# MP-Gadget/shenqi

Hardware: AMD Instinct MI355X
Metric: particle-steps/sec (grav+PM+SPH) at 256^3; rms force error vs ref (higher is better)
Workload: dtype f64

## Files before the change

include/shenqi_hip.h:

```cpp
#ifndef SHENQI_HIP_H
#define SHENQI_HIP_H

#include <stddef.h>
#include <stdint.h>

#ifdef __cplusplus
extern "C" {
#endif

#define SHQ_OK 0
#define SHQ_ERR_INVALID 1
#define SHQ_ERR_DEVICE 2
#define SHQ_ERR_NOMEM 3
#define SHQ_ERR_STATE 4
#define SHQ_ERR_NOCONV 5

#define SHQ_NGRAVTAB 512
#define SHQ_NMAXCHILD 8
#define SHQ_NODELISTLENGTH 4
#define SHQ_TIMEBINS 46

typedef struct shq_context shq_context;


// ... 371 lines not shown
int shq_bh_dynamics_download(shq_context *ctx, const shq_part_view *parts, const shq_bh_dyn_view *bh);
int shq_set_bh_reposition(shq_context *ctx, int enabled);
int shq_kick_bh(shq_context *ctx, const double gravkick[SHQ_TIMEBINS + 1], const int32_t *active, int64_t nactive);
int shq_grav_short_run(shq_context *ctx, const shq_grav_params *params, const int32_t *active,
                       int64_t nactive, int update_potential, int walk_mode);
int shq_grav_short_run_range(shq_context *ctx, const shq_grav_params *params, int64_t first, int64_t count,
                             int update_potential, int walk_mode);
int shq_set_walk_stats(shq_context *ctx, int level);
int shq_set_walk_launch(shq_context *ctx, int persist, int leaf_ring);
int shq_set_walk_sparse(shq_context *ctx, int enable);
int shq_walk_pair_lean(shq_context *ctx);
int shq_set_walk_overlap(shq_context *ctx, int mode);
int shq_set_walk_addr(shq_context *ctx, int mode);
int shq_walk_last_addr(shq_context *ctx, int *mode);
int shq_walk_addr32_fits(int64_t numnodes);
int shq_walk_pair_status(shq_context *ctx, int64_t *recovered_launches, int64_t *stack_high_water, int64_t *last_mopped_tasks);
int shq_set_walk_debug(shq_context *ctx, int pair_spin_max, int pair_stack_cap);
int shq_set_tree_debug(shq_context *ctx, int64_t initial_node_cap);
int shq_tree_build_attempts(shq_context *ctx, int *attempts);
int shq_direct_force_sample(shq_context *ctx, const double *sample_pos, int64_t ns, int64_t nsrc, double BoxSize, double G, double h,
                            int repeat, double *accel);
int shq_grav_short_download(shq_context *ctx, double (*accel)[3], double *potential,
                            int64_t *ninteractions, shq_walk_stats *stats);
typedef struct shq_grav_query {
    double Pos[3];
    int32_t NodeList[4];
    double OldAcc;
} shq_grav_query;
typedef struct shq_grav_result {
    double Acc[3];
    double Potential;
} shq_grav_result;
int shq_grav_short_secondary(shq_context *ctx, const shq_grav_params *params, const shq_grav_query *queries, int64_t nq,
                             shq_grav_result *results, int64_t *ninteractions, int update_potential);
typedef struct shq_data_index {
    int32_t Task;
    int32_t Index;
    int32_t NodeList[4];
// ... 980 lines not shown
```

shenqi_amd/capi.py:

```python
import ctypes as C
import os

import numpy as np

_HERE = os.path.dirname(os.path.abspath(__file__))
LIBDIR = os.environ.get("SHQ_LIBDIR") or os.path.join(_HERE, "lib")
DATADIR = os.path.join(_HERE, "data")

NGRAVTAB = 512
NMAXCHILD = 8
NOFIELD = C.c_size_t(-1).value

WALK_EXACT = 0
WALK_GROUP = 1
WALK_AUTO = 2
WALK_TREE_ORDER = 0x100
WALK_DEFER_POSTPROCESS = 0x200


class ShqError(RuntimeError):
    """Non-zero status from the library (the shim's endrun() equivalent)."""


def _load(name):
# ... 400 lines not shown
    getattr(hip, _f).restype = C.c_int
hip.shq_set_walk_stats.argtypes = [_vp, C.c_int]
hip.shq_set_walk_stats.restype = C.c_int
hip.shq_set_walk_launch.argtypes = [_vp, C.c_int, C.c_int]
hip.shq_set_walk_launch.restype = C.c_int
hip.shq_set_walk_sparse.argtypes = [_vp, C.c_int]
hip.shq_set_walk_sparse.restype = C.c_int
hip.shq_walk_pair_lean.argtypes = [_vp]
hip.shq_walk_pair_lean.restype = C.c_int
hip.shq_set_walk_overlap.argtypes = [_vp, C.c_int]
hip.shq_set_walk_overlap.restype = C.c_int
hip.shq_set_walk_addr.argtypes = [_vp, C.c_int]
hip.shq_set_walk_addr.restype = C.c_int
hip.shq_walk_last_addr.argtypes = [_vp, C.POINTER(C.c_int)]
hip.shq_walk_last_addr.restype = C.c_int
hip.shq_walk_addr32_fits.argtypes = [C.c_int64]
hip.shq_walk_addr32_fits.restype = C.c_int
hip.shq_pm_set_fft_transposed.argtypes = [_vp, C.c_int]
hip.shq_pm_set_fft_transposed.restype = C.c_int
hip.shq_walk_pair_status.argtypes = [_vp, C.POINTER(C.c_int64), C.POINTER(C.c_int64), C.POINTER(C.c_int64)]
hip.shq_walk_pair_status.restype = C.c_int
hip.shq_set_walk_debug.argtypes = [_vp, C.c_int, C.c_int]
hip.shq_set_walk_debug.restype = C.c_int
hip.shq_set_tree_debug.argtypes = [_vp, C.c_int64]
hip.shq_set_tree_debug.restype = C.c_int
hip.shq_tree_build_attempts.argtypes = [_vp, C.POINTER(C.c_int)]
hip.shq_tree_build_attempts.restype = C.c_int
hip.shq_direct_force_sample.argtypes = [_vp, _vp, C.c_int64, C.c_int64, C.c_double, C.c_double, C.c_double, C.c_int, _vp]
hip.shq_direct_force_sample.restype = C.c_int
hip.shq_exchange_plan.argtypes = [_vp, C.POINTER(ExchangeLayout), _vp, C.c_int64, _vp, C.c_int, C.c_int, C.c_int64, C.POINTER(C.c_int64), C.POINTER(C.c_int64), _vp]
# ... 926 lines not shown
```

shenqi_amd/csrc/capi.hip:

```cpp
#include "common.hpp"
#include <stdarg.h>
#include <string.h>
#include <stdlib.h>
#include <math.h>
#include <thread>
#include <atomic>
#include <algorithm>

static thread_local char g_err[1024] = "";

void shq_set_error(const char *fmt, ...)
{
    va_list ap;
    va_start(ap, fmt);
    vsnprintf(g_err, sizeof(g_err), fmt, ap);
    va_end(ap);
}

extern "C" const char *shq_last_error(void) { return g_err; }
extern "C" const char *shq_version(void) { return "shenqi_hip 0.1 (gfx950)"; }

namespace {

template <typename F> void parallel_for(int64_t n, F f)
// ... 144 lines not shown
                delete ctx;
                return SHQ_ERR_DEVICE;
            }
        }
    }
    if(const char *v = getenv("SHQ_PM_OVERLAP"))
        ctx->pm_overlap = atoi(v) != 0;
    if(const char *v = getenv("SHQ_PM_SCRUB"))
        ctx->pm_scrub = atoi(v) != 0;
    if(const char *v = getenv("SHQ_WALK_SPARSE"))
        ctx->walk_sparse = atoi(v);
    if(const char *v = getenv("SHQ_WALK_OVERLAP"))
        ctx->walk_overlap = atoi(v);
    if(const char *v = getenv("SHQ_WALK_ADDR"))
        ctx->walk_addr = atoi(v) != 0;
    if(const char *v = getenv("SHQ_TREE_TARGETS_REFRESH"))
        ctx->tree_targets_refresh = atoi(v) > 0 ? atoi(v) : 1;
    if(const char *v = getenv("SHQ_FFT_TRANSPOSED"))
        ctx->fft_transposed = atoi(v) != 0;
    if(const char *v = getenv("SHQ_TREEPM_FUSE"))
        ctx->treepm_fuse = atoi(v) != 0;
    if(const char *v = getenv("SHQ_WALK_VARIANT"))
        ctx->walk_variant = atoi(v);
    if(const char *v = getenv("SHQ_WALK_STATS_GUARD"))
        ctx->stats_guard = atoi(v);
    if(const char *v = getenv("SHQ_WALK_PADDING"))
        ctx->allow_padding = atoi(v) != 0;
    if(const char *v = getenv("SHQ_WALK_STATS"))
        ctx->walk_stats = atoi(v);
    if(const char *v = getenv("SHQ_XCD_K"))
// ... 112 lines not shown
}

extern "C" int shq_set_walk_overlap(shq_context *ctx, int mode)
{
    SHQ_CHECK(ctx, SHQ_ERR_INVALID, "null context");
    SHQ_CHECK(mode >= 0 && mode <= 2, SHQ_ERR_INVALID, "walk overlap mode %d", mode);
    ctx->walk_overlap = mode;
    return SHQ_OK;
}

extern "C" int shq_set_walk_addr(shq_context *ctx, int mode)
{
    SHQ_CHECK(ctx, SHQ_ERR_INVALID, "null context");
    SHQ_CHECK(mode == 0 || mode == 1, SHQ_ERR_INVALID, "walk addr mode %d", mode);
    ctx->walk_addr = mode;
    return SHQ_OK;
}

extern "C" int shq_walk_last_addr(shq_context *ctx, int *mode)
{
    SHQ_CHECK(ctx && mode, SHQ_ERR_INVALID, "null argument");
    *mode = ctx->last_walk_addr32 ? 1 : 0;
    return SHQ_OK;
}

extern "C" int shq_walk_pair_lean(shq_context *ctx)
{
    SHQ_CHECK(ctx, SHQ_ERR_INVALID, "null context");
    if(!ctx->node_lean_checked || !ctx->node_lean_bad.ptr)
        return 0;
// ... 604 lines not shown
{
    SHQ_CHECK(ctx && params, SHQ_ERR_INVALID, "null argument");
    SHQ_CHECK(ctx->have_parts && ctx->have_tree, SHQ_ERR_STATE, "grav_short_run: upload particles and tree first");
    SHQ_HIP(hipSetDevice(ctx->device));
    SHQ_TRY(shq_walk_check_status(ctx, false));
    const int32_t *d_active = nullptr;
    int64_t nt = 0;
    if((walk_mode & SHQ_WALK_TREE_ORDER) && !active) {
        SHQ_TRY(shq_build_tree_targets(ctx));
        d_active = ctx->tree_targets.ptr;
        nt = ctx->ntree_targets;
    } else
        SHQ_TRY(shq_resolve_active(ctx, active, nactive, ctx->nlocal, &d_active, &nt));
    const bool defer = (walk_mode & SHQ_WALK_DEFER_POSTPROCESS) != 0;
    walk_mode &= 0xff;
    SHQ_TRY(shq_launch_grav_walk(ctx, params, d_active, nt, update_potential, walk_mode));
    if(!defer)
        SHQ_TRY(shq_launch_grav_postprocess(ctx, params, d_active, nt, update_potential));
    ctx->grav_raw = defer;
    ctx->last_stats.ntargets = nt;
    return SHQ_OK;
}

extern "C" int shq_grav_short_run_range(shq_context *ctx, const shq_grav_params *params, int64_t first, int64_t count,
                                        int update_potential, int walk_mode)
{
    SHQ_CHECK(ctx && params, SHQ_ERR_INVALID, "null argument");
    SHQ_CHECK(ctx->have_parts && ctx->have_tree, SHQ_ERR_STATE, "grav_short_run_range: upload particles and tree first");
    const int64_t nown = ctx->nlocal;
    SHQ_CHECK(first >= 0 && count >= 0 && first + count <= nown, SHQ_ERR_INVALID, "grav_short_run_range: [%ld, +%ld) outside the %ld own particles",
              (long) first, (long) count, (long) nown);
    SHQ_CHECK((walk_mode & ~0xff) == 0, SHQ_ERR_INVALID, "grav_short_run_range: walk_mode flags are not supported");
    SHQ_HIP(hipSetDevice(ctx->device));
    hipStream_t main = ctx->stream;
    if(ctx->stream_walk) {
        SHQ_HIP(hipEventRecord(ctx->ev_walk_in, main));
        SHQ_HIP(hipStreamWaitEvent(ctx->stream_walk, ctx->ev_walk_in, 0));
        ctx->stream = ctx->stream_walk;
    }
    int rc = shq_launch_grav_walk(ctx, params, nullptr, count, update_potential, walk_mode, first);
    if(rc == SHQ_OK)
        rc = shq_launch_grav_postprocess(ctx, params, nullptr, count, update_potential, first);
    ctx->stream = main;
    if(ctx->stream_walk) {
        SHQ_HIP(hipEventRecord(ctx->ev_walk_out, ctx->stream_walk));
        SHQ_HIP(hipStreamWaitEvent(main, ctx->ev_walk_out, 0));
    }
    SHQ_TRY(rc);
    ctx->grav_raw = false;
    ctx->last_stats.ntargets = first == 0 ? count : ctx->last_stats.ntargets + count;
    return SHQ_OK;
}

namespace {
__global__ void grav_reduce_kernel(long long n, const int32_t *__restrict__ place, const shq_grav_result *__restrict__ res, double *acc,
// ... 63 lines not shown
    SHQ_HIP(hipStreamSynchronize(ctx->stream));
    return SHQ_OK;
}

extern "C" int shq_grav_postprocess(shq_context *ctx, const shq_grav_params *params, const int32_t *active, int64_t nactive,
                                    int update_potential)
{
    SHQ_CHECK(ctx && params, SHQ_ERR_INVALID, "null argument");
    SHQ_CHECK(ctx->have_parts && ctx->grav_raw, SHQ_ERR_STATE, "grav_postprocess: no deferred walk result on the device");
    SHQ_HIP(hipSetDevice(ctx->device));
    const int32_t *d_active = nullptr;
    int64_t nt = 0;
    SHQ_TRY(shq_resolve_active(ctx, active, nactive, ctx->nlocal, &d_active, &nt));
    SHQ_TRY(shq_launch_grav_postprocess(ctx, params, d_active, nt, update_potential));
    ctx->grav_raw = false;
    return SHQ_OK;
}

extern "C" int shq_grav_short_download(shq_context *ctx, double (*accel)[3], double *potential,
                                       int64_t *ninteractions, shq_walk_stats *stats)
{
    SHQ_CHECK(ctx, SHQ_ERR_INVALID, "null context");
    SHQ_CHECK(ctx->have_parts, SHQ_ERR_STATE, "nothing to download");
    SHQ_HIP(hipSetDevice(ctx->device));
    SHQ_TRY(shq_walk_check_status(ctx, true));
    const int64_t n = ctx->numpart;
    if(accel && n > 0)
        SHQ_HIP(hipMemcpyAsync(accel, ctx->acc.ptr, sizeof(double) * 3 * n, hipMemcpyDeviceToHost, ctx->stream));
    if(potential && n > 0)
        SHQ_HIP(hipMemcpyAsync(potential, ctx->pot.ptr, sizeof(double) * n, hipMemcpyDeviceToHost, ctx->stream));
// ... 270 lines not shown
    bool oldacc_done = ctx->pm_prestarted_oldacc;
    if(!prestarted) {
        ctx->readout_oldacc_G = (!fuse && ctx->numpart > 0 && ctx->treeacc.ptr && ctx->oldacc.ptr) ? params->G : 0.0;
        oldacc_done = ctx->readout_oldacc_G > 0;
        const int rc_pm = shq_pm_execute(ctx, pm, !fuse);
        ctx->readout_oldacc_G = 0;
        SHQ_TRY(rc_pm);
    }
    if(!fuse) {
        if(!oldacc_done)
            SHQ_TRY(shq_grav_refresh_oldacc(ctx, params->G));
    } else {
        ctx->fuse_G = params->G;
        ctx->fuse_readout = true;
    }
    const int rc = shq_launch_grav_walk(ctx, params, d_targets, n, update_potential, SHQ_WALK_EXACT);
    ctx->fuse_readout = false;
    SHQ_TRY(rc);
    SHQ_TRY(shq_launch_grav_postprocess(ctx, params, d_targets, n, update_potential));
    ctx->grav_raw = false;
    ctx->last_stats.ntargets = n;
    ctx->last_step_fused = fuse;
    return SHQ_OK;
}

extern "C" int shq_treepm_set_fuse(shq_context *ctx, int enable)
{
    SHQ_CHECK(ctx, SHQ_ERR_INVALID, "null context");
    ctx->treepm_fuse = enable != 0;
    return SHQ_OK;
}

// ... 143 lines not shown
```

shenqi_amd/csrc/common.hpp:

```cpp
#ifndef SHQ_COMMON_HPP
#define SHQ_COMMON_HPP

#include <hip/hip_runtime.h>
#include <hipfft/hipfft.h>
#include <stdint.h>
#include <stdio.h>
#include <string>
#include <vector>
#include "../../include/shenqi_hip.h"
#include "yields_math.hpp"
#include "cooling_math.hpp"

void shq_set_error(const char *fmt, ...);
void shq_heiii_run_free(shq_context *ctx);

#define SHQ_HIP(call)                                                                          \
    do {                                                                                       \
        hipError_t e_ = (call);                                                                \
        if(e_ != hipSuccess) {                                                                 \
            shq_set_error("%s:%d: %s failed: %s", __FILE__, __LINE__, #call, hipGetErrorString(e_)); \
            return (e_ == hipErrorOutOfMemory) ? SHQ_ERR_NOMEM : SHQ_ERR_DEVICE;               \
        }                                                                                      \
    } while(0)

// ... 414 lines not shown
    int walk_ring = 1;
    int num_cus = 256;
    DevBuf<unsigned int> walk_tasks;
    DevBuf<int4> sp_items, sp_stack;
    DevBuf<int32_t> sp_count;
    DevBuf<int> sp_flags;
    PinBuf<int> sp_host;
    int sp_stack_cap = 0;
    unsigned sp_spin_max = 0;
    int walk_sparse = 1;
    DevBuf<int> node_lean_bad;
    bool node_lean_checked = false;
    int walk_overlap = 1;
    int walk_addr = 1;
    bool last_walk_addr32 = false;
    bool sp_check_pending = false;
    int xcd_k = 32;
    float last_walk_ms = 0;
    int last_walk_mode = 0;

    PinBuf<char> stage;

    bool uvbg_keep = false;
    int uvbg_n = 0;
    std::vector<float> uvbg_j21, uvbg_xhi;
    double uvbg_ms[4] = {0, 0, 0, 0};
    DevBuf<double> uvbg_tw, uvbg_tabs, uvbg_part;
    DevBuf<int> uvbg_flag;
    int uvbg_tw_n = 0, uvbg_tabs_n = 0, uvbg_tabs_nr = 0;
    shq_heiii_stats heiii_stats = {};
// ... 59 lines not shown
__device__ inline long long shq_bh_ordinal(const int32_t *pidx, long long nbh, int32_t i)
{
    long long lo = 0, hi = nbh;
    while(lo < hi) {
        const long long mid = (lo + hi) >> 1;
        if(pidx[mid] < i)
            lo = mid + 1;
        else
            hi = mid;
    }
    return (lo < nbh && pidx[lo] == i) ? lo : -1;
}
int shq_resolve_active(shq_context *ctx, const int32_t *active, int64_t nactive, int64_t n_all, const int32_t **d_active, int64_t *nt);
int shq_launch_grav_walk(shq_context *ctx, const shq_grav_params *p, const int32_t *d_active,
                         int64_t ntargets, int update_potential, int walk_mode, int64_t first = 0);
int shq_launch_grav_postprocess(shq_context *ctx, const shq_grav_params *p, const int32_t *d_active,
                                int64_t ntargets, int update_potential, int64_t first = 0);
int shq_launch_oldacc(shq_context *ctx, double G);
void shq_launch_stats_init(shq_context *ctx);
void shq_fill_node_walk_params(shq_context *ctx, const shq_grav_params *p);
int shq_walk_reserve_sparse(shq_context *ctx, long long nwaves);
int shq_walk_check_status(shq_context *ctx, bool sync);
int shq_walk_prereserve(shq_context *ctx);
const int *shq_walk_error_word(shq_context *ctx);
int shq_launch_grav_walk_group(shq_context *ctx, const shq_grav_params *p, const int32_t *d_active, int64_t ntargets, int update_potential,
                               int64_t first);
int shq_launch_grav_walk_ghosts(shq_context *ctx, const shq_grav_params *p, const double4 *d_qpos, const double *d_qoldacc,
                                const int32_t *d_qstart, int64_t nq, double *d_acc, double *d_pot, int32_t *d_nint, int update_potential);
int shq_pm_execute(shq_context *ctx, const shq_pm_params *pm, bool readout = true);
int shq_pm_execute_forward(shq_context *ctx, const shq_pm_params *pm);
// ... 204 lines not shown
```

shenqi_amd/csrc/grav_group.hip:

```cpp
#include "common.hpp"
#include <algorithm>

namespace {

constexpr int GS = 8;
constexpr int WAVES = 4;
constexpr int STACK_CAP = 1280;
constexpr int STACK_SOFT = 1024;
constexpr int AMB_CAP = 128;
constexpr int FR_CAP = 512;
constexpr int CH = 512;

enum { ACT_T2, ACT_T1 };

struct ListArgs {
    const NodeG *G;
    const float4 *F;
    const double4 *posm;
    const double *oldacc;
    const int32_t *targets;
    long long ntargets;
    int root;
    double Box, invBox;
    double rcut, rcut2, bh2;
// ... 763 lines not shown
    *reinterpret_cast<int4 *>(&F[4 * i + 3]) = make_int4(kid[4], kid[5], kid[6], kid[7]);
}

__global__ void add_tests_kernel(GravStatsDev *s, const unsigned long long *ntests) { s->nvisited += *ntests; }

}

int shq_launch_grav_walk_group(shq_context *ctx, const shq_grav_params *p, const int32_t *d_active, int64_t ntargets, int update_potential,
                               int64_t first)
{
    SHQ_CHECK(first >= 0 && (first == 0 || !d_active) && first + ntargets <= ctx->numpart, SHQ_ERR_INVALID,
              "grav walk: bad target range [%ld, +%ld)", (long) first, (long) ntargets);
    SHQ_CHECK(ctx->have_parts && ctx->have_tree, SHQ_ERR_STATE, "grav walk: particles and tree must be uploaded first");
    SHQ_CHECK(p->ForceSoftening > 0 && p->cellsize > 0 && p->dx > 0, SHQ_ERR_INVALID, "grav params: softening/cellsize/dx must be > 0");
    SHQ_CHECK(ntargets >= 0 && ntargets <= ctx->numpart, SHQ_ERR_INVALID, "grav walk: ntargets %ld out of range", (long) ntargets);
    SHQ_TRY(ctx->gravtab.reserve(2 * SHQ_NGRAVTAB));
    SHQ_TRY(ctx->gstats.reserve(1));
    SHQ_TRY(ctx->walk_counters.reserve(4));
    SHQ_HIP(hipMemcpyAsync(ctx->gravtab.ptr, p->shortrange_table, sizeof(float) * SHQ_NGRAVTAB, hipMemcpyHostToDevice, ctx->stream));
    SHQ_HIP(hipMemcpyAsync(ctx->gravtab.ptr + SHQ_NGRAVTAB, p->shortrange_table_potential, sizeof(float) * SHQ_NGRAVTAB,
                           hipMemcpyHostToDevice, ctx->stream));
    if(first == 0)
        shq_launch_stats_init(ctx);
    if(ntargets == 0)
        return SHQ_OK;
    shq_fill_node_walk_params(ctx, p);
    const long long nn = ctx->numnodes;
    if(!ctx->have_group_aux) {
        SHQ_TRY(ctx->nodeF.reserve(4 * (size_t) (nn + 1)));
        node_t1_kernel<<<dim3((unsigned) ((nn + 255) / 256)), dim3(256), 0, ctx->stream>>>(ctx->nodeG.ptr, nn, ctx->nodeF.ptr);
        SHQ_HIP(hipGetLastError());
        ctx->have_group_aux = true;
    }
    if(ctx->walk_pool_chunks == 0) {
        size_t free_b = 0, total_b = 0;
        SHQ_HIP(hipMemGetInfo(&free_b, &total_b));
// ... 123 lines not shown
```

shenqi_amd/csrc/grav_walk.hip:

```cpp
#include "common.hpp"
#include "pm_readout.hpp"
#include <utility>
#include <stdlib.h>

namespace {

struct WalkArgs {
    const NodeG *nodeG;
    const double4 *posm;
    const double4 *posm_leaf;
    const double *oldacc;
    const int32_t *targets;
    const int32_t *qstart;
    double *acc;
    double *pot;
    int32_t *nint;
    GravStatsDev *stats;
    long long ntargets;
    int root;
    double Box, invBox, halfBox;
    double rcut, rcut2;
    double h, h2, h_inv, h3_inv;
    double inv_celldx;
    double errtol, bh2;
// ... 12 lines not shown
    int pmN, pmzp;
    double pmcell, pmffac, G;
    const double *treeacc;
    const uint8_t *pflags;
    double *gravpm, *pmpot, *oldacc_out;
    int4 *sp_items;
    int32_t *sp_count;
    int4 *sp_stack;
    int *sp_flags;
    int sp_stack_cap;
    unsigned sp_spin_max;
    int sp_mop;
    unsigned int *sp_task;
    int sp_live;
    const int *sp_lean_bad;
};

__device__ __forceinline__ double wrapd(double d, double L, double invL)
{
    return fma(-L, rint(d * invL), d);
}

__device__ __forceinline__ double rsqrt_fast(double x)
{
    const double y0 = __builtin_amdgcn_rsq(x);
    const double e = fma(-x * y0, y0, 1.0);
    return fma(y0 * e, fma(e, 0.375, 0.5), y0);
}

__device__ __forceinline__ double sconst(double c)
// ... 516 lines not shown
}

struct LeanProducts { double rcuthl, mlen2, inside, wraplim; };
__device__ __forceinline__ LeanProducts lean_products(double mass, double len, double rcut, double Box)
{
    LeanProducts r;
    const double hl = 0.5 * len;
    r.rcuthl = rcut + hl;
    r.mlen2 = mass * len * len;
    r.inside = 0.6 * len;
    r.wraplim = fmax(0.5 * Box - hl, 0.0);
    return r;
}
__device__ __forceinline__ int lean_level(double rootlen, double len) { return (__double2hiint(rootlen) - __double2hiint(len)) >> 20; }

#pragma clang diagnostic push
#pragma clang diagnostic ignored "-Wpass-failed"
template <bool POT, int WAVES>
__device__ __forceinline__ void grav_pair_body(const WalkArgs &a)
{
    __shared__ double4 tab[SHQ_NGRAVTAB];
    __shared__ double4 tgt_all[WAVES][64];
    __shared__ double acc_all[WAVES][4][64];
    __shared__ int cnt_all[WAVES][64];
    __shared__ double bh_lvl[32];
    if(a.sp_mop && agent_load(a.sp_flags + SP_GAVEUP) == 0)
        return;
    const double rootlen = a.Box * 1.001;
    if(threadIdx.x < 32) {
        const double l = ldexp(rootlen, -(int) threadIdx.x);
// ... 215 lines not shown
                push_leaves(ob.leaf0, ob.leafn, pb.slot);
            sp_high = sp > sp_high ? sp : sp_high;
            if(sp > a.sp_stack_cap - 1280) {
                if(lane == 0) {
                    agent_store(a.sp_flags + SP_OVERFLOW, 1);
                    atomicOr(a.sp_flags + SP_STICKY_ERROR, 1);
                }
                sp = 0;
            }
            __builtin_amdgcn_fence(__ATOMIC_RELEASE, "wavefront");
            __builtin_amdgcn_wave_barrier();
        }
        long long nint = 0;
        if(have) {
            nint = agent_load(&a.nint[pi]);
            if(cnt > 0) {
                __builtin_amdgcn_fence(__ATOMIC_ACQUIRE, "wavefront");
                a.acc[3 * pi + 0] = agent_load(&a.acc[3 * pi + 0]) + acc[0][lane];
                a.acc[3 * pi + 1] = agent_load(&a.acc[3 * pi + 1]) + acc[1][lane];
                a.acc[3 * pi + 2] = agent_load(&a.acc[3 * pi + 2]) + acc[2][lane];
                if(POT)
                    a.pot[pi] = agent_load(&a.pot[pi]) + acc[3][lane];
                nint += (long long) cntl[lane];
                a.nint[pi] = (int32_t) nint;
            }
        }
        long long mn = have ? nint : 0x7fffffffffffll, mx = have ? nint : 0, sm = have ? nint : 0;
        for(int off = 32; off > 0; off >>= 1) {
            const long long o1 = __shfl_xor(mn, off), o2 = __shfl_xor(mx, off), o3 = __shfl_xor(sm, off);
            mn = o1 < mn ? o1 : mn;
            mx = o2 > mx ? o2 : mx;
            sm += o3;
        }
        w_sum += sm;
        w_min = mn < w_min ? mn : w_min;
        w_max = mx > w_max ? mx : w_max;
        if(lane == 0)
            agent_store(&a.sp_count[task], (int32_t) SP_TASK_DONE);
        __builtin_amdgcn_wave_barrier();
// ... 75 lines not shown
            M = fmin(M, fmin(g[i].center[k] - hl, Box - (g[i].center[k] + hl)));
        const double wl = fmax(0.5 * Box - hl, 0.0);
        g[i].wraplim = (len > 0 && wl > 0 && M >= rcut + 1.5 * len) ? -wl : wl;
        if(lean_bad && i < n - 1) {
            const double rootlen = Box * 1.001;
            const int k = lean_level(rootlen, len);
            const LeanProducts lp = lean_products(g[i].mass, len, rcut, Box);
            const bool ok = len > 0 && k >= 0 && k < 32 && ldexp(rootlen, -k) == len && lp.rcuthl == g[i].rcuthl &&
                            lp.mlen2 == g[i].mlen2 && lp.inside == g[i].inside && lp.wraplim == wl;
            if(!ok)
                *lean_bad = 1;
        }
    }
}

__global__ void stats_init_kernel(GravStatsDev *s)
{
    s->ninteractions = 0;
    s->nvisited = 0;
    s->nwave_applies = 0;
    s->nwave_node_applies = 0;
    s->nnode_interactions = 0;
    s->min_int = 0x7fffffffffffll;
    s->max_int = 0;
    for(int b = 0; b < 8; b++)
        s->hist_visit[b] = s->hist_node[b] = s->hist_leaf[b] = 0;
    for(int b = 0; b < 4; b++)
        s->lonely[b] = 0;
}

template <bool POT, bool PREFETCH, int LEAFB, bool BH>
bool launch_variant_bh(int stats, bool persist, dim3 grid, dim3 block, hipStream_t stream, const WalkArgs &a, size_t dyn_lds = 0, bool addr32 = false)
{
    constexpr bool RO = !PREFETCH && LEAFB == 2 && !BH;
    if(a.pm_mesh && a.sp_items && RO && !stats && persist && block.x == 512)
        grav_walk_exact_kernel<POT, PREFETCH, LEAFB, 0, BH, false, RO, RO, RO, RO><<<grid, block, dyn_lds, stream>>>(a);
    else if(a.sp_items && RO && !stats && persist && block.x == 512 && addr32) {
        grav_walk_exact_kernel<POT, PREFETCH, LEAFB, 0, BH, false, RO, RO, false, RO, RO><<<grid, block, dyn_lds, stream>>>(a);
        return true;
    } else if(a.sp_items && RO && !stats && persist && block.x == 512)
        grav_walk_exact_kernel<POT, PREFETCH, LEAFB, 0, BH, false, RO, RO, false, RO><<<grid, block, dyn_lds, stream>>>(a);
    else if(a.pm_mesh && RO && !stats && persist && block.x == 512)
        grav_walk_exact_kernel<POT, PREFETCH, LEAFB, 0, BH, false, RO, RO, RO><<<grid, block, dyn_lds, stream>>>(a);
// ... 13 lines not shown
}

template <bool POT, bool PREFETCH, int LEAFB>
bool launch_variant(int stats, bool persist, dim3 grid, dim3 block, hipStream_t stream, const WalkArgs &a, size_t dyn_lds = 0, bool addr32 = false)
{
    if(a.useBH)
        return launch_variant_bh<POT, PREFETCH, LEAFB, true>(stats, persist, grid, block, stream, a, dyn_lds, addr32);
    return launch_variant_bh<POT, PREFETCH, LEAFB, false>(stats, persist, grid, block, stream, a, dyn_lds, addr32);
}

}

extern "C" int shq_walk_addr32_fits(int64_t numnodes) { return (numnodes >= 0 && numnodes + 1 <= ((int64_t) 1 << 25)) ? 1 : 0; }

void shq_launch_stats_init(shq_context *ctx) { stats_init_kernel<<<1, 1, 0, ctx->stream>>>(ctx->gstats.ptr); }

void shq_fill_node_walk_params(shq_context *ctx, const shq_grav_params *p)
{
    if((ctx->node_rcut != p->Rcut || ctx->node_bh2 != p->BHOpeningAngle2) && ctx->numnodes > 0) {
        const long long n = ctx->numnodes + 1;
        int *lean_bad = nullptr;
        if(ctx->node_lean_bad.reserve(16) == SHQ_OK && hipMemsetAsync(ctx->node_lean_bad.ptr, 0, sizeof(int) * 16, ctx->stream) == hipSuccess)
            lean_bad = ctx->node_lean_bad.ptr;
        ctx->node_lean_checked = lean_bad != nullptr;
        fill_rcuthl_kernel<<<dim3((unsigned) ((n + 255) / 256)), dim3(256), 0, ctx->stream>>>(ctx->nodeG.ptr, n, p->Rcut, p->BHOpeningAngle2, p->BoxSize, lean_bad);
        ctx->node_rcut = p->Rcut;
        ctx->node_bh2 = p->BHOpeningAngle2;
    }
}

// ... 37 lines not shown
    a.pmN = a.pmzp = 0;
    a.pmcell = a.pmffac = a.G = 0;
    a.treeacc = nullptr;
    a.pflags = nullptr;
    a.gravpm = a.pmpot = a.oldacc_out = nullptr;
    a.sp_items = nullptr;
    a.sp_count = nullptr;
    a.sp_stack = nullptr;
    a.sp_flags = nullptr;
    a.sp_stack_cap = SHQ_SPARSE_STACK;
    a.sp_spin_max = SHQ_SPARSE_SPIN;
    a.sp_mop = 0;
    a.sp_lean_bad = nullptr;
    a.sp_live = 0;
    a.sp_task = nullptr;
    a.nwaves = 0;
    a.task_run_log2 = 7;
}

int shq_launch_grav_walk_ghosts(shq_context *ctx, const shq_grav_params *p, const double4 *d_qpos, const double *d_qoldacc,
                                const int32_t *d_qstart, int64_t nq, double *d_acc, double *d_pot, int32_t *d_nint, int update_potential)
{
    SHQ_CHECK(ctx->have_tree, SHQ_ERR_STATE, "secondary walk: no tree");
    SHQ_CHECK(p->ForceSoftening > 0 && p->cellsize > 0 && p->dx > 0, SHQ_ERR_INVALID, "grav params: softening/cellsize/dx must be > 0");
    SHQ_TRY(ctx->gravtab.reserve(2 * SHQ_NGRAVTAB));
    SHQ_TRY(ctx->gstats.reserve(1));
    SHQ_HIP(hipMemcpyAsync(ctx->gravtab.ptr, p->shortrange_table, sizeof(float) * SHQ_NGRAVTAB, hipMemcpyHostToDevice, ctx->stream));
    SHQ_HIP(hipMemcpyAsync(ctx->gravtab.ptr + SHQ_NGRAVTAB, p->shortrange_table_potential, sizeof(float) * SHQ_NGRAVTAB,
                           hipMemcpyHostToDevice, ctx->stream));
    stats_init_kernel<<<1, 1, 0, ctx->stream>>>(ctx->gstats.ptr);
    if(nq == 0)
        return SHQ_OK;
    WalkArgs a;
    fill_walk_args(ctx, p, a);
    a.posm = d_qpos;
    a.oldacc = d_qoldacc;
    a.qstart = d_qstart;
    a.acc = d_acc;
    a.pot = d_pot;
    a.nint = d_nint;
    a.ntargets = nq;
    const long long nwaves = (nq + 63) / 64;
    const dim3 grid((unsigned) ((nwaves + 3) / 4)), block(256);
    if(update_potential) {
// ... 103 lines not shown
    if(recovered_launches)
        *recovered_launches = w[SP_STICKY_RECOVERED];
    if(stack_high_water)
        *stack_high_water = w[SP_STICKY_HIGHWATER];
    if(last_mopped_tasks)
        *last_mopped_tasks = w[SP_MOPPED];
    return shq_walk_check_status(ctx, true);
}

int shq_launch_grav_walk(shq_context *ctx, const shq_grav_params *p, const int32_t *d_active, int64_t ntargets,
                         int update_potential, int walk_mode, int64_t first)
{
    if(walk_mode == SHQ_WALK_AUTO)
        walk_mode = (d_active && ntargets * 10 < ctx->ntreeparts) ? SHQ_WALK_GROUP : SHQ_WALK_EXACT;
    ctx->last_walk_mode = walk_mode;
    if(walk_mode == SHQ_WALK_GROUP)
        return shq_launch_grav_walk_group(ctx, p, d_active, ntargets, update_potential, first);
    SHQ_CHECK(first >= 0 && (first == 0 || !d_active) && (first + ntargets <= ctx->numpart || (d_active && ctx->allow_padding)), SHQ_ERR_INVALID,
              "grav walk: bad target range [%ld, +%ld)", (long) first, (long) ntargets);
    SHQ_CHECK(ctx->have_parts && ctx->have_tree, SHQ_ERR_STATE, "grav walk: particles and tree must be uploaded first");
    SHQ_CHECK(walk_mode == SHQ_WALK_EXACT, SHQ_ERR_INVALID, "unknown walk_mode %d", walk_mode);
    SHQ_CHECK(p->ForceSoftening > 0 && p->cellsize > 0 && p->dx > 0, SHQ_ERR_INVALID, "grav params: softening/cellsize/dx must be > 0");
    SHQ_CHECK(ntargets >= 0 && (ntargets <= ctx->numpart || (d_active && ctx->allow_padding)), SHQ_ERR_INVALID, "grav walk: ntargets %ld out of range", (long) ntargets);
    SHQ_TRY(ctx->gravtab.reserve(2 * SHQ_NGRAVTAB));
    SHQ_TRY(ctx->gstats.reserve(1));
    SHQ_HIP(hipMemcpyAsync(ctx->gravtab.ptr, p->shortrange_table, sizeof(float) * SHQ_NGRAVTAB, hipMemcpyHostToDevice, ctx->stream));
    SHQ_HIP(hipMemcpyAsync(ctx->gravtab.ptr + SHQ_NGRAVTAB, p->shortrange_table_potential, sizeof(float) * SHQ_NGRAVTAB,
                           hipMemcpyHostToDevice, ctx->stream));
    if(first == 0)
        stats_init_kernel<<<1, 1, 0, ctx->stream>>>(ctx->gstats.ptr);
    if(ntargets == 0)
        return SHQ_OK;

    WalkArgs a;
    fill_walk_args(ctx, p, a);
    a.targets = d_active;
    a.ntargets = ntargets;
    a.posm += first;
    a.oldacc += first;
    a.acc += 3 * first;
    a.pot += first;
    a.nint += first;

    const int threads = 256;
    const long long nwaves = (ntargets + 63) / 64;
    const long long blocks = (nwaves + (threads / 64) - 1) / (threads / 64);
    SHQ_CHECK(blocks < (1ll << 31), SHQ_ERR_INVALID, "grav walk: too many targets for one launch");
    const int variant = ctx->walk_variant;
    const int stats = ctx->walk_stats;
    static const int bpc_env = getenv("SHQ_WALK_BLOCKS_PER_CU") ? atoi(getenv("SHQ_WALK_BLOCKS_PER_CU")) : 8;
    const int bpc = bpc_env >= 1 && bpc_env <= 8 ? bpc_env : 8;
    const bool persist = ctx->walk_persist && !stats && variant == 3 && (ctx->walk_persist == 2 || blocks > (long long) ctx->num_cus * bpc);
    const bool ring = persist && ctx->walk_ring && bpc == 8;
    const bool sparse = ring && ctx->walk_sparse && !p->TreeUseBH;
    const bool live = sparse && ctx->walk_overlap && !ctx->pm_overlap && ctx->stream_pair && ctx->ev_pair_fork && ctx->ev_pair_join && !stats &&
                      (ctx->walk_overlap == 2 || nwaves >= (long long) ctx->num_cus * 32 * 4);
    const long long pair_blocks = (long long) ctx->num_cus * (live ? 4 : SHQ_PAIR_WG_PER_CU);
    const long long mop_blocks = (long long) ctx->num_cus * SHQ_PAIR_WG_PER_CU;
    if(sparse) {
        SHQ_TRY(shq_walk_reserve_sparse(ctx, nwaves));
        SHQ_HIP(hipMemsetAsync(ctx->sp_flags.ptr, 0, sizeof(int) * SP_STICKY_ERROR, ctx->stream));
        SHQ_HIP(hipMemsetAsync(ctx->sp_flags.ptr + SP_TASK_COUNTER, 0, sizeof(int) * 16, ctx->stream));
        a.sp_items = ctx->sp_items.ptr;
        a.sp_count = ctx->sp_count.ptr;
        a.sp_stack = ctx->sp_stack.ptr;
        a.sp_flags = ctx->sp_flags.ptr;
        a.sp_stack_cap = ctx->sp_stack_cap;
        a.sp_spin_max = ctx->sp_spin_max;
        a.sp_lean_bad = ctx->node_lean_checked && ctx->walk_sparse != 2 ? ctx->node_lean_bad.ptr : nullptr;
        if(live) {
            SHQ_HIP(hipMemsetAsync(ctx->sp_count.ptr, 0xff, sizeof(int32_t) * (size_t) nwaves, ctx->stream));
            a.sp_live = 1;
        }
        a.sp_task = reinterpret_cast<unsigned int *>(ctx->sp_flags.ptr + SP_TASK_COUNTER);
        a.nwaves = nwaves;
    }
    long long launch_blocks = blocks;
    size_t dyn_lds = 0;
    if(persist) {
        SHQ_TRY(ctx->walk_tasks.reserve(8 * 16));
        SHQ_HIP(hipMemsetAsync(ctx->walk_tasks.ptr, 0, sizeof(unsigned int) * 8 * 16, ctx->stream));
        a.task_counters = ctx->walk_tasks.ptr;
        a.nwaves = nwaves;
        int lg = 0;
        while((1u << lg) < 4u * (a.xcdK ? a.xcdK : 1u))
            lg++;
        a.task_run_log2 = lg;
        const long long wpb = ring ? 8 : 4;
        const long long need = (nwaves + wpb - 1) / wpb, resident = (long long) ctx->num_cus * (ring ? (live ? 3 : 4) : bpc);
        launch_blocks = need < resident ? need : resident;
        if(bpc < 8)
            dyn_lds = (size_t) ((160 * 1024 / bpc - 16384) / 1024 * 1024 - 1024);
        if(ring)
            dyn_lds = sizeof(double4) * SHQ_LEAF_RING * 8;
    }
    bool scrubbed = false, swap_meshes = false;
// ... 71 lines not shown
        if(live) {
            SHQ_HIP(hipEventRecord(ctx->ev_pair_join, ps));
            SHQ_HIP(hipStreamWaitEvent(ctx->stream, ctx->ev_pair_join, 0));
            WalkArgs m = a;
            m.sp_live = 0;
            m.sp_mop = 1;
            const dim3 mg((unsigned) mop_blocks);
            if(update_potential)
                grav_pair_kernel<true><<<mg, dim3(64 * SHQ_PAIR_WAVES), 0, ctx->stream>>>(m);
            else
                grav_pair_kernel<false><<<mg, dim3(64 * SHQ_PAIR_WAVES), 0, ctx->stream>>>(m);
            SHQ_HIP(hipGetLastError());
        }
        SHQ_HIP(hipMemcpyAsync(ctx->sp_host.ptr, ctx->sp_flags.ptr + SP_STICKY_ERROR, sizeof(int) * 8, hipMemcpyDeviceToHost, ctx->stream));
        ctx->sp_check_pending = true;
    }
    SHQ_HIP(hipEventRecord(ctx->ev_end[SHQ_T_WALK], ctx->stream));
    if(swap_meshes) {
        std::swap(ctx->mesh.ptr, ctx->mesh_alt.ptr);
        std::swap(ctx->mesh.cap, ctx->mesh_alt.cap);
    }
    if(scrubbed)
        ctx->mesh_zeroed = true;
    return SHQ_OK;
}

int shq_launch_grav_postprocess(shq_context *ctx, const shq_grav_params *p, const int32_t *d_active, int64_t ntargets,
                                int update_potential, int64_t first)
{
    if(ntargets == 0)
        return SHQ_OK;
    const int threads = 256;
    const long long blocks = (ntargets + threads - 1) / threads;
    grav_postprocess_kernel<<<dim3((unsigned) blocks), dim3(threads), 0, ctx->stream>>>(
        d_active, ntargets, ctx->posm.ptr + first, ctx->acc.ptr + 3 * first, ctx->pot.ptr + first, ctx->treeacc.ptr + 3 * first, p->G,
        p->ForceSoftening, p->cbrtrho0, update_potential);
    SHQ_HIP(hipGetLastError());
    return SHQ_OK;
}

namespace {
__global__ __launch_bounds__(256) void direct_sample_kernel(const double *__restrict__ tpos, int ns, const double4 *__restrict__ posm,
                                                            long long nsrc, long long chunk, double Box, double G, double h, int repeat,
                                                            double *__restrict__ out)
// ... 88 lines not shown
```

Before: 440.4 million.

## Fuse gravity postprocess into sparse pair-walk writeback and cache gravtab uploads

When the sparse pair walk is followed by postprocessing, the walk's final per-particle writeback now applies the G scaling, stores the tree acceleration and finishes the potential in the same pass. The separate postprocess kernel is then skipped. Several memsets and the stats init are merged into a single reset kernel, and the short-range table upload is skipped when the host copy is unchanged. The aim is to remove a full pass over the acc/pot arrays plus a few small launches and H2D copies, at the cost of more complex writeback logic that now depends on the finish flag and on caller state.

```diff
diff --git a/include/shenqi_hip.h b/include/shenqi_hip.h
--- a/include/shenqi_hip.h
+++ b/include/shenqi_hip.h
@@ -409,6 +409,8 @@
 int shq_set_walk_addr(shq_context *ctx, int mode);
 int shq_walk_last_addr(shq_context *ctx, int *mode);
 int shq_walk_addr32_fits(int64_t numnodes);
+int shq_set_walk_finish(shq_context *ctx, int enable);
+int shq_walk_last_finish(shq_context *ctx, int *finish);
 int shq_walk_pair_status(shq_context *ctx, int64_t *recovered_launches, int64_t *stack_high_water, int64_t *last_mopped_tasks);
 int shq_set_walk_debug(shq_context *ctx, int pair_spin_max, int pair_stack_cap);
 int shq_set_tree_debug(shq_context *ctx, int64_t initial_node_cap);
@@ -417,6 +419,7 @@
                             int repeat, double *accel);
 int shq_grav_short_download(shq_context *ctx, double (*accel)[3], double *potential,
                             int64_t *ninteractions, shq_walk_stats *stats);
+int shq_grav_tree_accel_download(shq_context *ctx, double (*tree_accel)[3]);
 typedef struct shq_grav_query {
     double Pos[3];
     int32_t NodeList[4];
diff --git a/shenqi_amd/capi.py b/shenqi_amd/capi.py
--- a/shenqi_amd/capi.py
+++ b/shenqi_amd/capi.py
@@ -438,6 +438,12 @@
 hip.shq_set_walk_addr.restype = C.c_int
 hip.shq_walk_last_addr.argtypes = [_vp, C.POINTER(C.c_int)]
 hip.shq_walk_last_addr.restype = C.c_int
+hip.shq_grav_tree_accel_download.argtypes = [_vp, _vp]
+hip.shq_grav_tree_accel_download.restype = C.c_int
+hip.shq_set_walk_finish.argtypes = [_vp, C.c_int]
+hip.shq_set_walk_finish.restype = C.c_int
+hip.shq_walk_last_finish.argtypes = [_vp, C.POINTER(C.c_int)]
+hip.shq_walk_last_finish.restype = C.c_int
 hip.shq_walk_addr32_fits.argtypes = [C.c_int64]
 hip.shq_walk_addr32_fits.restype = C.c_int
 hip.shq_pm_set_fft_transposed.argtypes = [_vp, C.c_int]
diff --git a/shenqi_amd/csrc/capi.hip b/shenqi_amd/csrc/capi.hip
--- a/shenqi_amd/csrc/capi.hip
+++ b/shenqi_amd/csrc/capi.hip
@@ -182,6 +182,8 @@
         ctx->walk_overlap = atoi(v);
     if(const char *v = getenv("SHQ_WALK_ADDR"))
         ctx->walk_addr = atoi(v) != 0;
+    if(const char *v = getenv("SHQ_WALK_FINISH"))
+        ctx->walk_finish = atoi(v) != 0;
     if(const char *v = getenv("SHQ_TREE_TARGETS_REFRESH"))
         ctx->tree_targets_refresh = atoi(v) > 0 ? atoi(v) : 1;
     if(const char *v = getenv("SHQ_FFT_TRANSPOSED"))
@@ -324,6 +326,21 @@
     SHQ_CHECK(ctx, SHQ_ERR_INVALID, "null context");
     SHQ_CHECK(mode == 0 || mode == 1, SHQ_ERR_INVALID, "walk addr mode %d", mode);
     ctx->walk_addr = mode;
+    return SHQ_OK;
+}
+
+extern "C" int shq_set_walk_finish(shq_context *ctx, int enable)
+{
+    SHQ_CHECK(ctx, SHQ_ERR_INVALID, "null context");
+    SHQ_CHECK(enable == 0 || enable == 1, SHQ_ERR_INVALID, "walk finish %d", enable);
+    ctx->walk_finish = enable;
+    return SHQ_OK;
+}
+
+extern "C" int shq_walk_last_finish(shq_context *ctx, int *finish)
+{
+    SHQ_CHECK(ctx && finish, SHQ_ERR_INVALID, "null argument");
+    *finish = ctx->last_walk_finish;
     return SHQ_OK;
 }
 
@@ -958,7 +975,10 @@
         SHQ_TRY(shq_resolve_active(ctx, active, nactive, ctx->nlocal, &d_active, &nt));
     const bool defer = (walk_mode & SHQ_WALK_DEFER_POSTPROCESS) != 0;
     walk_mode &= 0xff;
-    SHQ_TRY(shq_launch_grav_walk(ctx, params, d_active, nt, update_potential, walk_mode));
+    ctx->postprocess_follows = !defer;
+    const int rc_walk = shq_launch_grav_walk(ctx, params, d_active, nt, update_potential, walk_mode);
+    ctx->postprocess_follows = false;
+    SHQ_TRY(rc_walk);
     if(!defer)
         SHQ_TRY(shq_launch_grav_postprocess(ctx, params, d_active, nt, update_potential));
     ctx->grav_raw = defer;
@@ -982,7 +1002,9 @@
         SHQ_HIP(hipStreamWaitEvent(ctx->stream_walk, ctx->ev_walk_in, 0));
         ctx->stream = ctx->stream_walk;
     }
+    ctx->postprocess_follows = true;
     int rc = shq_launch_grav_walk(ctx, params, nullptr, count, update_potential, walk_mode, first);
+    ctx->postprocess_follows = false;
     if(rc == SHQ_OK)
         rc = shq_launch_grav_postprocess(ctx, params, nullptr, count, update_potential, first);
     ctx->stream = main;
@@ -1076,6 +1098,17 @@
     SHQ_TRY(shq_resolve_active(ctx, active, nactive, ctx->nlocal, &d_active, &nt));
     SHQ_TRY(shq_launch_grav_postprocess(ctx, params, d_active, nt, update_potential));
     ctx->grav_raw = false;
+    return SHQ_OK;
+}
+
+extern "C" int shq_grav_tree_accel_download(shq_context *ctx, double (*tree_accel)[3])
+{
+    SHQ_CHECK(ctx && tree_accel, SHQ_ERR_INVALID, "null argument");
+    SHQ_CHECK(ctx->have_parts, SHQ_ERR_STATE, "nothing to download");
+    SHQ_HIP(hipSetDevice(ctx->device));
+    if(ctx->numpart > 0)
+        SHQ_HIP(hipMemcpyAsync(tree_accel, ctx->treeacc.ptr, sizeof(double) * 3 * ctx->numpart, hipMemcpyDeviceToHost, ctx->stream));
+    SHQ_HIP(hipStreamSynchronize(ctx->stream));
     return SHQ_OK;
 }
 
@@ -1376,8 +1409,10 @@
         ctx->fuse_G = params->G;
         ctx->fuse_readout = true;
     }
+    ctx->postprocess_follows = true;
     const int rc = shq_launch_grav_walk(ctx, params, d_targets, n, update_potential, SHQ_WALK_EXACT);
     ctx->fuse_readout = false;
+    ctx->postprocess_follows = false;
     SHQ_TRY(rc);
     SHQ_TRY(shq_launch_grav_postprocess(ctx, params, d_targets, n, update_potential));
     ctx->grav_raw = false;
diff --git a/shenqi_amd/csrc/common.hpp b/shenqi_amd/csrc/common.hpp
--- a/shenqi_amd/csrc/common.hpp
+++ b/shenqi_amd/csrc/common.hpp
@@ -452,6 +452,12 @@
     int walk_overlap = 1;
     int walk_addr = 1;
     bool last_walk_addr32 = false;
+    int walk_finish = 1;
+    bool postprocess_follows = false;
+    bool walk_finished = false;
+    int last_walk_finish = 0;
+    float gravtab_host[2 * SHQ_NGRAVTAB] = {};
+    const float *gravtab_dev = nullptr;
     bool sp_check_pending = false;
     int xcd_k = 32;
     float last_walk_ms = 0;
@@ -541,6 +547,7 @@
 int shq_resolve_active(shq_context *ctx, const int32_t *active, int64_t nactive, int64_t n_all, const int32_t **d_active, int64_t *nt);
 int shq_launch_grav_walk(shq_context *ctx, const shq_grav_params *p, const int32_t *d_active,
                          int64_t ntargets, int update_potential, int walk_mode, int64_t first = 0);
+int shq_upload_gravtab(shq_context *ctx, const shq_grav_params *p);
 int shq_launch_grav_postprocess(shq_context *ctx, const shq_grav_params *p, const int32_t *d_active,
                                 int64_t ntargets, int update_potential, int64_t first = 0);
 int shq_launch_oldacc(shq_context *ctx, double G);
diff --git a/shenqi_amd/csrc/grav_group.hip b/shenqi_amd/csrc/grav_group.hip
--- a/shenqi_amd/csrc/grav_group.hip
+++ b/shenqi_amd/csrc/grav_group.hip
@@ -801,12 +801,9 @@
     SHQ_CHECK(ctx->have_parts && ctx->have_tree, SHQ_ERR_STATE, "grav walk: particles and tree must be uploaded first");
     SHQ_CHECK(p->ForceSoftening > 0 && p->cellsize > 0 && p->dx > 0, SHQ_ERR_INVALID, "grav params: softening/cellsize/dx must be > 0");
     SHQ_CHECK(ntargets >= 0 && ntargets <= ctx->numpart, SHQ_ERR_INVALID, "grav walk: ntargets %ld out of range", (long) ntargets);
-    SHQ_TRY(ctx->gravtab.reserve(2 * SHQ_NGRAVTAB));
+    SHQ_TRY(shq_upload_gravtab(ctx, p));
     SHQ_TRY(ctx->gstats.reserve(1));
     SHQ_TRY(ctx->walk_counters.reserve(4));
-    SHQ_HIP(hipMemcpyAsync(ctx->gravtab.ptr, p->shortrange_table, sizeof(float) * SHQ_NGRAVTAB, hipMemcpyHostToDevice, ctx->stream));
-    SHQ_HIP(hipMemcpyAsync(ctx->gravtab.ptr + SHQ_NGRAVTAB, p->shortrange_table_potential, sizeof(float) * SHQ_NGRAVTAB,
-                           hipMemcpyHostToDevice, ctx->stream));
     if(first == 0)
         shq_launch_stats_init(ctx);
     if(ntargets == 0)
diff --git a/shenqi_amd/csrc/grav_walk.hip b/shenqi_amd/csrc/grav_walk.hip
--- a/shenqi_amd/csrc/grav_walk.hip
+++ b/shenqi_amd/csrc/grav_walk.hip
@@ -2,6 +2,7 @@
 #include "pm_readout.hpp"
 #include <utility>
 #include <stdlib.h>
+#include <string.h>
 
 namespace {
 
@@ -50,6 +51,9 @@
     unsigned int *sp_task;
     int sp_live;
     const int *sp_lean_bad;
+    int finish;
+    double fin_G, fin_cbrtrho0;
+    double *fin_treeacc;
 };
 
 __device__ __forceinline__ double wrapd(double d, double L, double invL)
@@ -596,6 +600,15 @@
 }
 __device__ __forceinline__ int lean_level(double rootlen, double len) { return (__double2hiint(rootlen) - __double2hiint(len)) >> 20; }
 
+__device__ __attribute__((noinline)) double finish_potential(double p, double m, double h, double cbrtrho0, double G)
+{
+#pragma clang fp contract(off)
+    p += m / (h / 2.8);
+    p = fma(-cbrtrho0, 2.8372975 * pow(m, 2.0 / 3), p);
+    p *= G;
+    return p;
+}
+
 #pragma clang diagnostic push
 #pragma clang diagnostic ignored "-Wpass-failed"
 template <bool POT, int WAVES>
@@ -841,15 +854,37 @@
         long long nint = 0;
         if(have) {
             nint = agent_load(&a.nint[pi]);
-            if(cnt > 0) {
-                __builtin_amdgcn_fence(__ATOMIC_ACQUIRE, "wavefront");
-                a.acc[3 * pi + 0] = agent_load(&a.acc[3 * pi + 0]) + acc[0][lane];
-                a.acc[3 * pi + 1] = agent_load(&a.acc[3 * pi + 1]) + acc[1][lane];
-                a.acc[3 * pi + 2] = agent_load(&a.acc[3 * pi + 2]) + acc[2][lane];
+            if(cnt > 0 || a.finish) {
+                if(cnt > 0)
+                    __builtin_amdgcn_fence(__ATOMIC_ACQUIRE, "wavefront");
+                double r0 = agent_load(&a.acc[3 * pi + 0]), r1 = agent_load(&a.acc[3 * pi + 1]), r2 = agent_load(&a.acc[3 * pi + 2]);
+                double rp = POT ? agent_load(&a.pot[pi]) : 0.0;
+                if(cnt > 0) {
+                    r0 = r0 + acc[0][lane];
+                    r1 = r1 + acc[1][lane];
+                    r2 = r2 + acc[2][lane];
+                    if(POT)
+                        rp = rp + acc[3][lane];
+                    nint += (long long) cntl[lane];
+                    a.nint[pi] = (int32_t) nint;
+                }
+                if(a.finish) {
+#pragma clang fp contract(off)
+                    r0 = r0 * a.fin_G;
+                    r1 = r1 * a.fin_G;
+                    r2 = r2 * a.fin_G;
+                    if(POT && a.finish == 2) {
+                        a.fin_treeacc[3 * pi + 0] = r0;
+                        a.fin_treeacc[3 * pi + 1] = r1;
+                        a.fin_treeacc[3 * pi + 2] = r2;
+                        rp = finish_potential(rp, a.posm[pi].w, a.h, a.fin_cbrtrho0, a.fin_G);
+                    }
+                }
+                a.acc[3 * pi + 0] = r0;
+                a.acc[3 * pi + 1] = r1;
+                a.acc[3 * pi + 2] = r2;
                 if(POT)
-                    a.pot[pi] = agent_load(&a.pot[pi]) + acc[3][lane];
-                nint += (long long) cntl[lane];
-                a.nint[pi] = (int32_t) nint;
+                    a.pot[pi] = rp;
             }
         }
         long long mn = have ? nint : 0x7fffffffffffll, mx = have ? nint : 0, sm = have ? nint : 0;
@@ -955,7 +990,7 @@
     }
 }
 
-__global__ void stats_init_kernel(GravStatsDev *s)
+__device__ __forceinline__ void stats_reset(GravStatsDev *s)
 {
     s->ninteractions = 0;
     s->nvisited = 0;
@@ -968,6 +1003,21 @@
         s->hist_visit[b] = s->hist_node[b] = s->hist_leaf[b] = 0;
     for(int b = 0; b < 4; b++)
         s->lonely[b] = 0;
+}
+
+__global__ void stats_init_kernel(GravStatsDev *s) { stats_reset(s); }
+
+__global__ __launch_bounds__(128) void walk_reset_kernel(int *sp_flags, unsigned int *walk_tasks, GravStatsDev *s)
+{
+    const int i = threadIdx.x;
+    if(i < SP_STICKY_ERROR)
+        sp_flags[i] = 0;
+    if(i < 16)
+        sp_flags[SP_TASK_COUNTER + i] = 0;
+    if(i < 8 * 16)
+        walk_tasks[i] = 0u;
+    if(i == 0 && s)
+        stats_reset(s);
 }
 
 template <bool POT, bool PREFETCH, int LEAFB, bool BH>
@@ -1011,6 +1061,22 @@
 extern "C" int shq_walk_addr32_fits(int64_t numnodes) { return (numnodes >= 0 && numnodes + 1 <= ((int64_t) 1 << 25)) ? 1 : 0; }
 
 void shq_launch_stats_init(shq_context *ctx) { stats_init_kernel<<<1, 1, 0, ctx->stream>>>(ctx->gstats.ptr); }
+
+int shq_upload_gravtab(shq_context *ctx, const shq_grav_params *p)
+{
+    const size_t half = sizeof(float) * SHQ_NGRAVTAB;
+    SHQ_TRY(ctx->gravtab.reserve(2 * SHQ_NGRAVTAB));
+    if(ctx->gravtab_dev == ctx->gravtab.ptr && memcmp(ctx->gravtab_host, p->shortrange_table, half) == 0 &&
+       memcmp(ctx->gravtab_host + SHQ_NGRAVTAB, p->shortrange_table_potential, half) == 0)
+        return SHQ_OK;
+    ctx->gravtab_dev = nullptr;
+    SHQ_HIP(hipMemcpyAsync(ctx->gravtab.ptr, p->shortrange_table, half, hipMemcpyHostToDevice, ctx->stream));
+    SHQ_HIP(hipMemcpyAsync(ctx->gravtab.ptr + SHQ_NGRAVTAB, p->shortrange_table_potential, half, hipMemcpyHostToDevice, ctx->stream));
+    memcpy(ctx->gravtab_host, p->shortrange_table, half);
+    memcpy(ctx->gravtab_host + SHQ_NGRAVTAB, p->shortrange_table_potential, half);
+    ctx->gravtab_dev = ctx->gravtab.ptr;
+    return SHQ_OK;
+}
 
 void shq_fill_node_walk_params(shq_context *ctx, const shq_grav_params *p)
 {
@@ -1078,6 +1144,9 @@
     a.sp_lean_bad = nullptr;
     a.sp_live = 0;
     a.sp_task = nullptr;
+    a.finish = 0;
+    a.fin_G = a.fin_cbrtrho0 = 0;
+    a.fin_treeacc = nullptr;
     a.nwaves = 0;
     a.task_run_log2 = 7;
 }
@@ -1087,11 +1156,8 @@
 {
     SHQ_CHECK(ctx->have_tree, SHQ_ERR_STATE, "secondary walk: no tree");
     SHQ_CHECK(p->ForceSoftening > 0 && p->cellsize > 0 && p->dx > 0, SHQ_ERR_INVALID, "grav params: softening/cellsize/dx must be > 0");
-    SHQ_TRY(ctx->gravtab.reserve(2 * SHQ_NGRAVTAB));
+    SHQ_TRY(shq_upload_gravtab(ctx, p));
     SHQ_TRY(ctx->gstats.reserve(1));
-    SHQ_HIP(hipMemcpyAsync(ctx->gravtab.ptr, p->shortrange_table, sizeof(float) * SHQ_NGRAVTAB, hipMemcpyHostToDevice, ctx->stream));
-    SHQ_HIP(hipMemcpyAsync(ctx->gravtab.ptr + SHQ_NGRAVTAB, p->shortrange_table_potential, sizeof(float) * SHQ_NGRAVTAB,
-                           hipMemcpyHostToDevice, ctx->stream));
     stats_init_kernel<<<1, 1, 0, ctx->stream>>>(ctx->gstats.ptr);
     if(nq == 0)
         return SHQ_OK;
@@ -1225,6 +1291,8 @@
     if(walk_mode == SHQ_WALK_AUTO)
         walk_mode = (d_active && ntargets * 10 < ctx->ntreeparts) ? SHQ_WALK_GROUP : SHQ_WALK_EXACT;
     ctx->last_walk_mode = walk_mode;
+    ctx->walk_finished = false;
+    ctx->last_walk_finish = 0;
     if(walk_mode == SHQ_WALK_GROUP)
         return shq_launch_grav_walk_group(ctx, p, d_active, ntargets, update_potential, first);
     SHQ_CHECK(first >= 0 && (first == 0 || !d_active) && (first + ntargets <= ctx->numpart || (d_active && ctx->allow_padding)), SHQ_ERR_INVALID,
@@ -1233,15 +1301,13 @@
     SHQ_CHECK(walk_mode == SHQ_WALK_EXACT, SHQ_ERR_INVALID, "unknown walk_mode %d", walk_mode);
     SHQ_CHECK(p->ForceSoftening > 0 && p->cellsize > 0 && p->dx > 0, SHQ_ERR_INVALID, "grav params: softening/cellsize/dx must be > 0");
     SHQ_CHECK(ntargets >= 0 && (ntargets <= ctx->numpart || (d_active && ctx->allow_padding)), SHQ_ERR_INVALID, "grav walk: ntargets %ld out of range", (long) ntargets);
-    SHQ_TRY(ctx->gravtab.reserve(2 * SHQ_NGRAVTAB));
+    SHQ_TRY(shq_upload_gravtab(ctx, p));
     SHQ_TRY(ctx->gstats.reserve(1));
-    SHQ_HIP(hipMemcpyAsync(ctx->gravtab.ptr, p->shortrange_table, sizeof(float) * SHQ_NGRAVTAB, hipMemcpyHostToDevice, ctx->stream));
-    SHQ_HIP(hipMemcpyAsync(ctx->gravtab.ptr + SHQ_NGRAVTAB, p->shortrange_table_potential, sizeof(float) * SHQ_NGRAVTAB,
-                           hipMemcpyHostToDevice, ctx->stream));
-    if(first == 0)
-        stats_init_kernel<<<1, 1, 0, ctx->stream>>>(ctx->gstats.ptr);
-    if(ntargets == 0)
+    if(ntargets == 0) {
+        if(first == 0)
+            stats_init_kernel<<<1, 1, 0, ctx->stream>>>(ctx->gstats.ptr);
         return SHQ_OK;
+    }
 
     WalkArgs a;
     fill_walk_args(ctx, p, a);
@@ -1270,8 +1336,15 @@
     const long long mop_blocks = (long long) ctx->num_cus * SHQ_PAIR_WG_PER_CU;
     if(sparse) {
         SHQ_TRY(shq_walk_reserve_sparse(ctx, nwaves));
-        SHQ_HIP(hipMemsetAsync(ctx->sp_flags.ptr, 0, sizeof(int) * SP_STICKY_ERROR, ctx->stream));
-        SHQ_HIP(hipMemsetAsync(ctx->sp_flags.ptr + SP_TASK_COUNTER, 0, sizeof(int) * 16, ctx->stream));
+        SHQ_TRY(ctx->walk_tasks.reserve(8 * 16));
+        walk_reset_kernel<<<1, 128, 0, ctx->stream>>>(ctx->sp_flags.ptr, ctx->walk_tasks.ptr, first == 0 ? ctx->gstats.ptr : nullptr);
+        SHQ_HIP(hipGetLastError());
+        if(ctx->walk_finish && ctx->postprocess_follows) {
+            a.finish = update_potential ? 2 : 1;
+            a.fin_G = p->G;
+            a.fin_cbrtrho0 = p->cbrtrho0;
+            a.fin_treeacc = ctx->treeacc.ptr + 3 * first;
+        }
         a.sp_items = ctx->sp_items.ptr;
         a.sp_count = ctx->sp_count.ptr;
         a.sp_stack = ctx->sp_stack.ptr;
@@ -1285,12 +1358,15 @@
         }
         a.sp_task = reinterpret_cast<unsigned int *>(ctx->sp_flags.ptr + SP_TASK_COUNTER);
         a.nwaves = nwaves;
-    }
+    } else if(first == 0)
+        stats_init_kernel<<<1, 1, 0, ctx->stream>>>(ctx->gstats.ptr);
     long long launch_blocks = blocks;
     size_t dyn_lds = 0;
     if(persist) {
-        SHQ_TRY(ctx->walk_tasks.reserve(8 * 16));
-        SHQ_HIP(hipMemsetAsync(ctx->walk_tasks.ptr, 0, sizeof(unsigned int) * 8 * 16, ctx->stream));
+        if(!sparse) {
+            SHQ_TRY(ctx->walk_tasks.reserve(8 * 16));
+            SHQ_HIP(hipMemsetAsync(ctx->walk_tasks.ptr, 0, sizeof(unsigned int) * 8 * 16, ctx->stream));
+        }
         a.task_counters = ctx->walk_tasks.ptr;
         a.nwaves = nwaves;
         int lg = 0;
@@ -1392,6 +1468,10 @@
         }
         SHQ_HIP(hipMemcpyAsync(ctx->sp_host.ptr, ctx->sp_flags.ptr + SP_STICKY_ERROR, sizeof(int) * 8, hipMemcpyDeviceToHost, ctx->stream));
         ctx->sp_check_pending = true;
+        if(a.finish) {
+            ctx->walk_finished = true;
+            ctx->last_walk_finish = a.finish;
+        }
     }
     SHQ_HIP(hipEventRecord(ctx->ev_end[SHQ_T_WALK], ctx->stream));
     if(swap_meshes) {
@@ -1406,6 +1486,10 @@
 int shq_launch_grav_postprocess(shq_context *ctx, const shq_grav_params *p, const int32_t *d_active, int64_t ntargets,
                                 int update_potential, int64_t first)
 {
+    if(ctx->walk_finished) {
+        ctx->walk_finished = false;
+        return SHQ_OK;
+    }
     if(ntargets == 0)
         return SHQ_OK;
     const int threads = 256;
```

Measured after the change: 443.8 million (median of 4 runs). No clear change (+0.8%).
